# shao-lab/MotifScan

Measured on NVIDIA B200. Metric: motif_bp_scored_per_sec_both_strands, higher is better.
Workload: dtype e4m3 x e4m3 -> f16 tensor-core prefilter + f64 exact

## Files before the change

### motifscan_b200/csrc/kernels.cuh

```cuda
#pragma once
#include "common.cuh"

namespace msb {

__device__ __forceinline__ int64_t find_seq(const int64_t *__restrict__ poff, int64_t n_seqs,
                                            int64_t p) {
    int64_t lo = 0, hi = n_seqs;
    while (hi - lo > 1) {
        int64_t mid = (lo + hi) >> 1;
        if (__ldg(poff + mid) <= p) lo = mid; else hi = mid;
    }
    return lo;
}

__device__ __forceinline__ int base_code(const SeqView &S, int64_t q) {
    uint32_t m = __ldg(S.nmask + (q >> 5));
    if ((m >> (q & 31)) & 1u) return -1;
    uint32_t w = __ldg(S.codes + (q >> 4));
    return (int) ((w >> ((q & 15) * 2)) & 3u);
}

__global__ void __launch_bounds__(256)
encode_pack_kernel(const uint8_t *__restrict__ ascii, const int64_t *__restrict__ seq_off,
                   const int64_t *__restrict__ poff, const int32_t *__restrict__ len,
// ... 323 lines not shown
            const float vf = pw32[4 * c + row], vr = *(rev_end - 4 * c - row);
            if (!((w.nmask >> c) & 1u)) { f32 += vf; r32 += vr; }
        }
        if (L > left) continue;
        const float floor32 = s_floor[kl];
        const bool try_f = (E.strand & 1) && !(f32 < floor32), try_r = (E.strand & 2) && !(r32 < floor32);
        if (try_f || try_r) {
            const uint32_t m = s_motif[kl];
            const double *pw = E.mot.pwm + 4 * (int64_t) __ldg(E.mot.col_off + m);
            if (try_f) test_and_emit(E, m, p, 0, exact_raw_w(w, pw, L, 0));
            if (try_r) test_and_emit(E, m, p, 1, exact_raw_w(w, pw, L, 1));
        }
    }
}

__global__ void __launch_bounds__(256)
decode_sites_kernel(SeqView S, const uint64_t *__restrict__ key, int64_t n, int key_shift,
                    int32_t *__restrict__ seq_idx, int32_t *__restrict__ start,
                    int8_t *__restrict__ strand) {
    int64_t i = (int64_t) blockIdx.x * blockDim.x + threadIdx.x;
    if (i >= n) return;
    const uint64_t k = key[i];
    const int64_t p = site_pos(k, key_shift);
    const int64_t s = __ldg(S.blk_seq + (p >> 5));
    seq_idx[i] = (int32_t) s;
    start[i] = (int32_t) (p - __ldg(S.poff + s));
    strand[i] = (int8_t) (key_rev(k) + 1);
}

__global__ void __launch_bounds__(256)
compact_sites_kernel(const uint64_t *__restrict__ key, int64_t n, int key_shift, uint32_t *__restrict__ out) {
    const int64_t i = (int64_t) blockIdx.x * blockDim.x + threadIdx.x;
    if (i < n) out[i] = (uint32_t) (key[i] & ((1ull << key_shift) - 1ull));
}

__global__ void __launch_bounds__(256)
motif_offsets_kernel(const uint64_t *__restrict__ key, int64_t n, int32_t n_motifs, int key_shift,
                     int64_t *__restrict__ offsets) {
    const int32_t m = blockIdx.x * blockDim.x + threadIdx.x;
    if (m > n_motifs) return;
    int64_t lo = 0, hi = n;
    while (lo < hi) {
        const int64_t mid = (lo + hi) >> 1;
        if ((int64_t) site_motif(__ldg(key + mid), key_shift) < (int64_t) m) lo = mid + 1; else hi = mid;
    }
    offsets[m] = lo;
}

__global__ void __launch_bounds__(256)
count_hits_kernel(const uint64_t *__restrict__ key, int64_t n, int key_shift, int32_t n_motifs, int in_smem,
                  unsigned long long *__restrict__ counts) {
    extern __shared__ unsigned int s_hist[];
    if (in_smem) {
        for (int32_t m = threadIdx.x; m < n_motifs; m += blockDim.x) s_hist[m] = 0;
        __syncthreads();
    }
    for (int64_t i = (int64_t) blockIdx.x * blockDim.x + threadIdx.x; i < n; i += (int64_t) gridDim.x * blockDim.x) {
        const uint32_t m = site_motif(__ldg(key + i), key_shift);
        if (in_smem) atomicAdd(s_hist + m, 1u); else atomicAdd(counts + m, 1ull);
    }
    if (in_smem) {
        __syncthreads();
        for (int32_t m = threadIdx.x; m < n_motifs; m += blockDim.x)
            if (s_hist[m]) atomicAdd(counts + m, (unsigned long long) s_hist[m]);
    }
}

__global__ void __launch_bounds__(256)
region_counts_kernel(const uint64_t *__restrict__ key, const int32_t *__restrict__ seq_idx, int64_t n,
                     int key_shift, unsigned long long *__restrict__ out) {
    const int64_t i = (int64_t) blockIdx.x * blockDim.x + threadIdx.x;
    if (i >= n) return;
    const uint32_t m = site_motif(key[i], key_shift);
    if (i == 0 || site_motif(key[i - 1], key_shift) != m || seq_idx[i - 1] != seq_idx[i]) atomicAdd(out + m, 1ull);
}

__global__ void __launch_bounds__(256)
dedup_flags_kernel(const uint64_t *__restrict__ key, const int32_t *__restrict__ seq_idx,
                   const int32_t *__restrict__ start, const int8_t *__restrict__ strand,
// ... 29 lines not shown
__global__ void __launch_bounds__(256)
scatter_kept_kernel(const int32_t *__restrict__ keep, const int64_t *__restrict__ dst, int64_t n,
                    const uint64_t *__restrict__ key, const double *__restrict__ score,
                    const int32_t *__restrict__ seq_idx, const int32_t *__restrict__ start,
                    const int8_t *__restrict__ strand, uint64_t *__restrict__ o_key,
                    double *__restrict__ o_score, int32_t *__restrict__ o_seq,
                    int32_t *__restrict__ o_start, int8_t *__restrict__ o_strand) {
    const int64_t i = (int64_t) blockIdx.x * blockDim.x + threadIdx.x;
    if (i >= n || !keep[i]) return;
    const int64_t j = dst[i];
    o_key[j] = key[i];
    o_score[j] = score[i];
    o_seq[j] = seq_idx[i];
    o_start[j] = start[i];
    o_strand[j] = strand[i];
}

__global__ void __launch_bounds__(256)
score0_kernel(SeqView S, MotifView M, int strand, int32_t m_begin, int32_t m_end, int64_t out_stride,
              double *__restrict__ out) {
    const int64_t i = (int64_t) blockIdx.x * blockDim.x + threadIdx.x;
    if (i >= S.n_seqs) return;
    const int64_t p = __ldg(S.poff + i);
    for (int32_t m = m_begin + (int32_t) blockIdx.y; m < m_end; m += (int32_t) gridDim.y) {
        const int L = __ldg(M.len + m);
        const double *pw = M.pwm + 4 * (int64_t) __ldg(M.col_off + m);
        double f = 0.0, r = 0.0;
        for (int c = 0; c < L; c++) {
            const int row = base_code(S, p + c);
            if (row >= 0) {
// ... 226 lines not shown
```

### motifscan_b200/csrc/msb200.cu

```cuda
#include <cub/cub.cuh>

#include <algorithm>
#include <cmath>
#include <cstdio>
#include <cstdlib>
#include <cstring>
#include <functional>
#include <limits>
#include <mutex>
#include <new>
#include <numeric>
#include <charconv>
#include <thread>

#include "kernels.cuh"
#include "prefilter_tc.cuh"

namespace msb {

static constexpr int kSelSmemKeys = 24576;

static thread_local std::string g_err;
void set_error(const std::string &msg) { g_err = msg; }
int cuda_fail(cudaError_t e, const char *what, const char *file, int line) {
// ... 31 lines not shown
using namespace msb;

struct msb_ctx {
    int device = 0;
    cudaStream_t stream = nullptr;
    bool own_stream = false;
    int sm_count = 0;
    cudaEvent_t ev[8] = {};
    cudaStream_t copy_stream = nullptr;
    cudaEvent_t slice_ev[8] = {};
    double t[MSB_T_COUNT] = {};
    int64_t c[MSB_C_COUNT] = {};
    DevBuf ascii, seq_off, cand, dirty, hit_key, hit_score, key_alt, score_alt, sort_tmp, counters;
    DevBuf out_seq, out_start, out_strand, scores, scores_sorted, seg_off, ranks, sel;
    DevBuf keep, keep_pos, motif_counts, sel_aux, limit1;
    DevBuf lane_count;
    DevBuf bnd_range, bnd_cnt, bnd_dst, bnd_motif, bnd_seq, bnd_start, bnd_score, bnd_strand, bnd_flags;
    int64_t last_boundary = -1;
    struct FinSet {
        DevBuf key, score, seq, start, strand, offsets;
        cudaEvent_t read_done = nullptr;
        bool pending = false;
    } fin[2];
    int fin_cur = 0;
    bool last_counts_only = false;
    bool last_compact = false;
    const msb_seqs *last_seqs = nullptr;
    cudaStream_t d2h_stream = nullptr;
    cudaStream_t aux_stream = nullptr;
    cudaEvent_t aux_fork = nullptr, aux_join = nullptr;
// ... 4 lines not shown
    unsigned long long *h_counters = nullptr;
    std::vector<PinnedBlock> pinned_free;
    std::mutex pinned_mu;
    std::vector<DevBuf> dev_free;
    std::mutex dev_mu;
    int64_t last_sites = 0;
    int32_t last_n_motifs = 0;
    int64_t last_n_seqs = 0;
    int last_key_shift = 0;
    int opt_tc_prof = 0;
    int opt_ascii_slices = 4;
    int opt_tc_first_lane_cap = 0;
    int opt_poison_pool = 0;
    int opt_tc_interleave = 1;
    int opt_select_pilot = 1;
};

struct TcTableSet {
    bool valid = false;
    uint64_t cutoff_version = 0;
    std::vector<int32_t> order;
    std::vector<int32_t> slow;
    std::vector<TcBatch> batches;
    int32_t lmax_fast = 0;
    int any_zero_hit = 0;
    DevBuf d_btab, d_col_info, d_len, d_order, d_slow;
};

struct msb_motifs {
    msb_ctx *ctx = nullptr;
// ... 189 lines not shown
                  std::to_string(prop.minor));
        return MSB_ECUDA;
    }
    msb_ctx *ctx = new (std::nothrow) msb_ctx();
    if (!ctx) { set_error("out of host memory"); return MSB_ENOMEM; }
    ctx->device = device;
    ctx->sm_count = prop.multiProcessorCount;
    if (stream) {
        ctx->stream = (cudaStream_t) stream;
    } else {
        cudaError_t se = cudaStreamCreateWithFlags(&ctx->stream, cudaStreamNonBlocking);
        if (se != cudaSuccess) { delete ctx; return cuda_fail(se, "cudaStreamCreate", __FILE__, __LINE__); }
        ctx->own_stream = true;
    }
    for (auto &evt : ctx->ev) cudaEventCreate(&evt);
    cudaHostAlloc((void **) &ctx->h_counters, 4 * sizeof(unsigned long long), cudaHostAllocDefault);
    if (ctx->counters.ensure(4 * sizeof(unsigned long long)) != MSB_OK || !ctx->h_counters) {
        msb_ctx_destroy(ctx);
        return MSB_ENOMEM;
    }
    ctx->opt_tc_prof = std::getenv("MSB_TC_PROF") ? 1 : 0;
    if (cudaStreamCreateWithFlags(&ctx->aux_stream, cudaStreamNonBlocking) != cudaSuccess ||
        cudaEventCreateWithFlags(&ctx->aux_fork, cudaEventDisableTiming) != cudaSuccess ||
        cudaEventCreateWithFlags(&ctx->aux_join, cudaEventDisableTiming) != cudaSuccess) {
        cudaGetLastError();
        if (ctx->aux_stream) cudaStreamDestroy(ctx->aux_stream);
        ctx->aux_stream = nullptr;
    }
    cudaFuncSetAttribute(prefilter_tc_kernel<false>, cudaFuncAttributeMaxDynamicSharedMemorySize, kTcSmemBytes);
    cudaFuncSetAttribute(prefilter_tc_kernel<true>, cudaFuncAttributeMaxDynamicSharedMemorySize, kTcSmemBytes);
    cudaFuncSetAttribute(select_ranks_kernel<true>, cudaFuncAttributeMaxDynamicSharedMemorySize, kSelSmemKeys * 8);
    cudaFuncSetAttribute(select_ranks_kernel<false>, cudaFuncAttributeMaxDynamicSharedMemorySize, kSelSmemKeys * 8);
    *out = ctx;
    return MSB_OK;
}

int msb_ctx_destroy(msb_ctx *ctx) {
    if (!ctx) return MSB_OK;
    cudaSetDevice(ctx->device);
    cudaStreamSynchronize(ctx->stream);
    for (DevBuf *b : {&ctx->ascii, &ctx->seq_off, &ctx->cand, &ctx->dirty, &ctx->hit_key, &ctx->hit_score,
                      &ctx->key_alt, &ctx->score_alt, &ctx->sort_tmp, &ctx->counters, &ctx->out_seq,
                      &ctx->out_start, &ctx->out_strand, &ctx->scores,
                      &ctx->scores_sorted, &ctx->seg_off, &ctx->ranks, &ctx->sel, &ctx->keep, &ctx->keep_pos,
                      &ctx->motif_counts, &ctx->sel_aux, &ctx->limit1, &ctx->lane_count, &ctx->bnd_range,
                      &ctx->bnd_cnt, &ctx->bnd_dst, &ctx->bnd_motif, &ctx->bnd_seq, &ctx->bnd_start, &ctx->bnd_score,
                      &ctx->bnd_strand, &ctx->bnd_flags})
        b->release();
    if (ctx->d2h_stream) cudaStreamSynchronize(ctx->d2h_stream);
    for (auto &f : ctx->fin) {
        for (DevBuf *b : {&f.key, &f.score, &f.seq, &f.start, &f.strand, &f.offsets}) b->release();
        if (f.read_done) cudaEventDestroy(f.read_done);
    }
    if (ctx->d2h_stream) cudaStreamDestroy(ctx->d2h_stream);
    if (ctx->aux_stream) { cudaStreamSynchronize(ctx->aux_stream); cudaStreamDestroy(ctx->aux_stream); }
    if (ctx->aux_fork) cudaEventDestroy(ctx->aux_fork);
    if (ctx->aux_join) cudaEventDestroy(ctx->aux_join);
    for (auto &b : ctx->pinned_free) cudaFreeHost(b.p);
    for (auto &b : ctx->dev_free) b.release();
    if (ctx->h_counters) cudaFreeHost(ctx->h_counters);
// ... 638 lines not shown
    MSB_TRY(T.d_slow.ensure(std::max<size_t>(T.slow.size() * 4, 16)));
    cudaStream_t st = ctx->stream;
    MSB_CUDA(cudaMemcpyAsync(T.d_btab.p, btab.data(), btab.size(), cudaMemcpyHostToDevice, st));
    MSB_CUDA(cudaMemcpyAsync(T.d_col_info.p, col_info.data(), col_info.size() * 4, cudaMemcpyHostToDevice, st));
    MSB_CUDA(cudaMemcpyAsync(T.d_len.p, tc_len.data(), tc_len.size() * 4, cudaMemcpyHostToDevice, st));
    if (!fast.empty()) MSB_CUDA(cudaMemcpyAsync(T.d_order.p, fast.data(), fast.size() * 4, cudaMemcpyHostToDevice, st));
    if (!T.slow.empty()) MSB_CUDA(cudaMemcpyAsync(T.d_slow.p, T.slow.data(), T.slow.size() * 4, cudaMemcpyHostToDevice, st));
    MSB_CUDA(cudaStreamSynchronize(st));
    T.cutoff_version = M->cutoff_version;
    T.valid = true;
    *out = &T;
    return MSB_OK;
}

static int read_counters(msb_ctx *ctx) {
    MSB_CUDA(cudaMemcpyAsync(ctx->h_counters, ctx->counters.p, 4 * sizeof(unsigned long long),
                             cudaMemcpyDeviceToHost, ctx->stream));
    MSB_CUDA(cudaStreamSynchronize(ctx->stream));
    return MSB_OK;
}

static int launch_positions(msb_ctx *ctx, const ExactParams &E, const int64_t *pos, int64_t n_pos, int64_t pos_base,
                            const int32_t *ids, int32_t n_ids) {
    if (n_pos <= 0 || n_ids <= 0) return MSB_OK;
    const int64_t max_threads = (int64_t) 1 << 38;
    const int64_t pos_per_launch = std::max<int64_t>(1, max_threads / n_ids);
    for (int64_t at = 0; at < n_pos; at += pos_per_launch) {
        const int64_t cnt = std::min(pos_per_launch, n_pos - at);
        const int64_t threads = cnt * n_ids;
        ExactParams e2 = E;
        if (pos) {
            exact_positions_kernel<<<(unsigned) ((threads + 255) / 256), 256, 0, ctx->stream>>>(e2, pos + at, cnt, 0, ids, n_ids);
        } else {
            exact_positions_kernel<<<(unsigned) ((threads + 255) / 256), 256, 0, ctx->stream>>>(e2, nullptr, cnt, pos_base + at, ids, n_ids);
        }
        MSB_CUDA(cudaGetLastError());
        ctx->c[MSB_C_LAUNCHES]++;
    }
    return MSB_OK;
}

typedef std::vector<std::pair<int64_t, int64_t>> RangeList;

static int make_ranges(const msb_seqs *S, int64_t n_ranges, const int64_t *r_seq, const int64_t *r_start,
                       const int64_t *r_end, RangeList *out) {
    if (n_ranges < 0 || (n_ranges > 0 && (!r_seq || !r_start || !r_end))) { set_error("msb_scan_ranges: bad ranges"); return MSB_EINVAL; }
    out->clear();
    for (int64_t i = 0; i < n_ranges; i++) {
        if (r_seq[i] < 0 || r_seq[i] >= S->n) { set_error("msb_scan_ranges: sequence index out of range"); return MSB_EINVAL; }
        if (r_start[i] < 0) { set_error("msb_scan_ranges: negative start"); return MSB_EINVAL; }
        const int64_t slen = S->seq_off[r_seq[i] + 1] - S->seq_off[r_seq[i]];
        const int64_t a = std::min(r_start[i], slen), b = std::min(r_end[i], slen);
        if (b > a) out->push_back({S->poff[r_seq[i]] + a, S->poff[r_seq[i]] + b});
// ... 142 lines not shown
        MSB_TRY(read_counters(ctx));
        n_rec = (int64_t) ctx->h_counters[0];
        n_dirty = (int64_t) ctx->h_counters[1];
        const int64_t worst = (int64_t) ctx->h_counters[3];
        const bool overflow = worst > lane_cap;
        if (!overflow && n_dirty <= dirty_cap) break;
        if (attempt >= 2) { set_error("msb_scan: candidate buffers kept overflowing"); return MSB_ENOMEM; }
        ctx->c[MSB_C_RETRIES]++;
        if (overflow) cand_cap = std::max(cand_cap, (worst + worst / 8 + 16) * 2 * n_lanes);
        dirty_cap = std::max(dirty_cap, n_dirty + n_dirty / 16 + 1024);
        MSB_CUDA(cudaEventRecord(ctx->ev[0], st));
    }
    ctx->c[MSB_C_CANDIDATES] = n_rec;
    ctx->c[MSB_C_DIRTY] = n_dirty;

    int64_t hit_cap = std::max<int64_t>(n_rec + n_rec / 4 + 1024, 1 << 16);
    if (n_dirty) hit_cap += std::min<int64_t>(n_dirty * 2 * std::max(n_fast, 1), 1 << 24);
    if (n_slow) hit_cap += 1 << 20;
    if (ctx->hit_key.cap / 8 > (size_t) hit_cap) hit_cap = (int64_t) (ctx->hit_key.cap / 8);
    int64_t n_hits = 0;
    for (int attempt = 0;; attempt++) {
        MSB_TRY(ctx->hit_key.ensure((size_t) hit_cap * 8));
        MSB_TRY(ctx->hit_score.ensure((size_t) hit_cap * 8));
        MSB_CUDA(cudaMemsetAsync(ctx->counters.as<unsigned long long>() + 2, 0, sizeof(unsigned long long), st));
        const bool forked = ctx->aux_stream && cudaEventRecord(ctx->aux_fork, st) == cudaSuccess;
        bool join_aux = false;
        ExactParams E;
        E.seq = sv;
        E.mot = mv;
        E.strand = strand;
        E.key_shift = key_shift;
        E.hit_key = ctx->hit_key.as<uint64_t>();
        E.hit_score = ctx->hit_score.as<double>();
        E.hit_cap = hit_cap;
        E.counters = ctx->counters.as<unsigned long long>();
// ... 13 lines not shown
            }
            ctx->c[MSB_C_LAUNCHES]++;
        }
        if (n_rec) {
            exact_records_kernel<<<(unsigned) (((int64_t) n_lanes * 32 + 255) / 256), 256, 0, st>>>(
                E, ctx->cand.as<uint4>(), lane_cap, ctx->lane_count.as<uint32_t>(), n_lanes, d_order,
                TT->d_col_info.as<uint32_t>());
            MSB_CUDA(cudaGetLastError());
            ctx->c[MSB_C_LAUNCHES]++;
        }
        if (join_aux) MSB_CUDA(cudaStreamWaitEvent(st, ctx->aux_join, 0));
        if (n_slow)
            for (auto &r : *ranges)
                MSB_TRY(launch_positions(ctx, E, nullptr, r.second - r.first, r.first, d_slow, n_slow));
        MSB_CUDA(cudaEventRecord(ctx->ev[2], st));
        MSB_TRY(read_counters(ctx));
        n_hits = (int64_t) ctx->h_counters[2];
        if (n_hits <= hit_cap) break;
        if (attempt >= 2) { set_error("msb_scan: hit buffers kept overflowing"); return MSB_ENOMEM; }
        ctx->c[MSB_C_RETRIES]++;
        hit_cap = n_hits + 1024;
    }
    ctx->c[MSB_C_HITS] = n_hits;

    int64_t n_final = n_hits;
    if (counts_only) {
        MSB_TRY(ctx->motif_counts.ensure((size_t) (M->n + 1) * 8));
        MSB_CUDA(cudaMemsetAsync(ctx->motif_counts.p, 0, (size_t) (M->n + 1) * 8, st));
        if (n_hits) {
            const bool in_smem = (size_t) M->n * 4 <= 40 * 1024;
            const unsigned grid = (unsigned) std::min<int64_t>((n_hits + 2047) / 2048, (int64_t) ctx->sm_count * 8);
            count_hits_kernel<<<grid, 256, in_smem ? (size_t) M->n * 4 : 0, st>>>(
                ctx->hit_key.as<uint64_t>(), n_hits, key_shift, M->n, in_smem ? 1 : 0, ctx->motif_counts.as<unsigned long long>());
            MSB_CUDA(cudaGetLastError());
            ctx->c[MSB_C_LAUNCHES]++;
        }
        size_t scan_bytes = 0;
        MSB_CUDA(cub::DeviceScan::ExclusiveSum(nullptr, scan_bytes, ctx->motif_counts.as<int64_t>(), F.offsets.as<int64_t>(), M->n + 1, st));
        MSB_TRY(ctx->sort_tmp.ensure(std::max<size_t>(scan_bytes, 16)));
        MSB_CUDA(cub::DeviceScan::ExclusiveSum(ctx->sort_tmp.p, scan_bytes, ctx->motif_counts.as<int64_t>(), F.offsets.as<int64_t>(), M->n + 1, st));
    } else if (n_hits) {
        const bool dedup = (flags & MSB_SCAN_DEDUP) != 0;
        if ((size_t) n_hits * 25 > ((size_t) 4 << 30)) {
            msb_ctx::FinSet &O = ctx->fin[fin_set ^ 1];
            if (O.pending) { MSB_CUDA(cudaEventSynchronize(O.read_done)); O.pending = false; }
            for (DevBuf *b : {&O.key, &O.score, &O.seq, &O.start, &O.strand}) b->release();
        }
        DevBuf &s_key = dedup ? ctx->key_alt : F.key, &s_score = dedup ? ctx->score_alt : F.score;
        DevBuf &s_seq = dedup ? ctx->out_seq : F.seq, &s_start = dedup ? ctx->out_start : F.start;
        DevBuf &s_strand = dedup ? ctx->out_strand : F.strand;
        MSB_TRY(s_key.ensure((size_t) n_hits * 8));
        MSB_TRY(s_score.ensure((size_t) n_hits * 8));
        MSB_TRY(s_seq.ensure((size_t) n_hits * 4));
        MSB_TRY(s_start.ensure((size_t) n_hits * 4));
        MSB_TRY(s_strand.ensure((size_t) n_hits));
        const int end_bit = key_shift + motif_bits;
        size_t tmp_bytes = 0;
        MSB_CUDA(cub::DeviceRadixSort::SortPairs(nullptr, tmp_bytes, ctx->hit_key.as<uint64_t>(), s_key.as<uint64_t>(),
                                                 ctx->hit_score.as<double>(), s_score.as<double>(), n_hits, 0, end_bit, st));
        MSB_TRY(ctx->sort_tmp.ensure(std::max<size_t>(tmp_bytes, 16)));
        MSB_CUDA(cub::DeviceRadixSort::SortPairs(ctx->sort_tmp.p, tmp_bytes, ctx->hit_key.as<uint64_t>(), s_key.as<uint64_t>(),
                                                 ctx->hit_score.as<double>(), s_score.as<double>(), n_hits, 0, end_bit, st));
        const unsigned grid = (unsigned) ((n_hits + 255) / 256);
        const bool compact = (flags & MSB_SCAN_COMPACT) && !dedup && key_shift <= 32;
        if (compact) {
            compact_sites_kernel<<<grid, 256, 0, st>>>(s_key.as<uint64_t>(), n_hits, key_shift, s_start.as<uint32_t>());
            ctx->last_compact = true;
        } else {
            decode_sites_kernel<<<grid, 256, 0, st>>>(sv, s_key.as<uint64_t>(), n_hits, key_shift, s_seq.as<int32_t>(),
                                                      s_start.as<int32_t>(), s_strand.as<int8_t>());
        }
        MSB_CUDA(cudaGetLastError());
        ctx->c[MSB_C_LAUNCHES] += 2;
        if (dedup) {
            MSB_TRY(ctx->keep.ensure((size_t) n_hits * 4));
            MSB_TRY(ctx->keep_pos.ensure((size_t) n_hits * 8));
            MSB_TRY(F.key.ensure((size_t) n_hits * 8));
            MSB_TRY(F.score.ensure((size_t) n_hits * 8));
            MSB_TRY(F.seq.ensure((size_t) n_hits * 4));
            MSB_TRY(F.start.ensure((size_t) n_hits * 4));
            MSB_TRY(F.strand.ensure((size_t) n_hits));
            dedup_flags_kernel<<<grid, 256, 0, st>>>(s_key.as<uint64_t>(), s_seq.as<int32_t>(), s_start.as<int32_t>(),
                                                     s_strand.as<int8_t>(), s_score.as<double>(),
                                                     n_hits, mv.len, key_shift, ctx->keep.as<int32_t>());
            MSB_CUDA(cudaGetLastError());
            size_t scan_bytes = 0;
            MSB_CUDA(cub::DeviceScan::ExclusiveSum(nullptr, scan_bytes, ctx->keep.as<int32_t>(), ctx->keep_pos.as<int64_t>(), n_hits, st));
            MSB_TRY(ctx->sort_tmp.ensure(std::max<size_t>(scan_bytes, 16)));
            MSB_CUDA(cub::DeviceScan::ExclusiveSum(ctx->sort_tmp.p, scan_bytes, ctx->keep.as<int32_t>(), ctx->keep_pos.as<int64_t>(), n_hits, st));
// ... 27 lines not shown
            int64_t n_boundary = 0;
            if (boundary && cells) {
                MSB_CUDA(chains(0));
                size_t bs = 0;
                MSB_CUDA(cub::DeviceScan::ExclusiveSum(nullptr, bs, ctx->bnd_cnt.as<int64_t>(), ctx->bnd_dst.as<int64_t>(), cells + 1, st));
                MSB_TRY(ctx->sort_tmp.ensure(std::max<size_t>(bs, 16)));
                MSB_CUDA(cub::DeviceScan::ExclusiveSum(ctx->sort_tmp.p, bs, ctx->bnd_cnt.as<int64_t>(), ctx->bnd_dst.as<int64_t>(), cells + 1, st));
                MSB_CUDA(cudaMemcpyAsync(&n_boundary, ctx->bnd_dst.as<int64_t>() + cells, 8, cudaMemcpyDeviceToHost, st));
            }
            int32_t last_keep = 0;
            int64_t last_pos = 0;
            MSB_CUDA(cudaMemcpyAsync(&last_keep, ctx->keep.as<int32_t>() + (n_hits - 1), 4, cudaMemcpyDeviceToHost, st));
            MSB_CUDA(cudaMemcpyAsync(&last_pos, ctx->keep_pos.as<int64_t>() + (n_hits - 1), 8, cudaMemcpyDeviceToHost, st));
            MSB_CUDA(cudaStreamSynchronize(st));
            n_final = last_pos + last_keep;
            if (n_boundary) {
                MSB_TRY(ctx->bnd_motif.ensure((size_t) n_boundary * 4));
                MSB_TRY(ctx->bnd_seq.ensure((size_t) n_boundary * 4));
                MSB_TRY(ctx->bnd_start.ensure((size_t) n_boundary * 4));
                MSB_TRY(ctx->bnd_score.ensure((size_t) n_boundary * 8));
                MSB_TRY(ctx->bnd_strand.ensure((size_t) n_boundary));
                MSB_TRY(ctx->bnd_flags.ensure((size_t) n_boundary));
                MSB_CUDA(chains(1));
                ctx->last_boundary = n_boundary;
            }
        }
        ctx->fin_key = F.key.as<uint64_t>();
        ctx->fin_score = F.score.as<double>();
        ctx->fin_seq = F.seq.as<int32_t>();
        ctx->fin_start = F.start.as<int32_t>();
        ctx->fin_strand = F.strand.as<int8_t>();
        motif_offsets_kernel<<<(unsigned) ((M->n + 1 + 255) / 256), 256, 0, st>>>(ctx->fin_key, n_final, M->n, key_shift,
                                                                                  F.offsets.as<int64_t>());
        MSB_CUDA(cudaGetLastError());
        ctx->c[MSB_C_LAUNCHES] += 1;
    }
    MSB_CUDA(cudaEventRecord(ctx->ev[3], st));
    MSB_CUDA(cudaStreamSynchronize(st));
    ctx->t[MSB_T_PREFILTER] = ev_ms(ctx->ev[0], ctx->ev[1]);
    ctx->t[MSB_T_EXACT] = ev_ms(ctx->ev[1], ctx->ev[2]);
    ctx->t[MSB_T_ORDER] = ev_ms(ctx->ev[2], ctx->ev[3]);
    ctx->t[MSB_T_D2H] = 0;
    ctx->last_sites = n_final;
    ctx->fin_cur = fin_set;
    ctx->last_counts_only = counts_only;
    return MSB_OK;
}

}

extern "C" {

int msb_ctx_set_option(msb_ctx *ctx, const char *name, int value) {
    if (!ctx) { set_error("msb_ctx_set_option: null ctx"); return MSB_EINVAL; }
    if (name && !std::strcmp(name, "tc_prof") && (value == 0 || value == 1)) { ctx->opt_tc_prof = value; return MSB_OK; }
    if (name && !std::strcmp(name, "tc_first_lane_cap") && value >= 0) { ctx->opt_tc_first_lane_cap = value; return MSB_OK; }
    if (name && !std::strcmp(name, "ascii_slices") && value >= 1 && value <= 7) { ctx->opt_ascii_slices = value; return MSB_OK; }
    if (name && !std::strcmp(name, "poison_pool") && (value == 0 || value == 1)) { ctx->opt_poison_pool = value; return MSB_OK; }
    if (name && !std::strcmp(name, "tc_interleave") && (value == 0 || value == 1)) { ctx->opt_tc_interleave = value; return MSB_OK; }
    if (name && !std::strcmp(name, "select_pilot") && (value == 0 || value == 1)) { ctx->opt_select_pilot = value; return MSB_OK; }
    set_error("msb_ctx_set_option: unknown option or value");
    return MSB_EINVAL;
}

int msb_scan_device(msb_ctx *ctx, const msb_motifs *M, const msb_seqs *S, int strand, int flags, int64_t *n_sites) {
    MSB_TRY(scan_device(ctx, const_cast<msb_motifs *>(M), S, strand, flags));
    if (n_sites) *n_sites = ctx->last_sites;
    return MSB_OK;
}

int msb_scan_device_counts(msb_ctx *ctx, int64_t *counts, int32_t n_motifs) {
    if (!ctx || (!counts && n_motifs)) { set_error("msb_scan_device_counts: null"); return MSB_EINVAL; }
    if (n_motifs != ctx->last_n_motifs) { set_error("msb_scan_device_counts: no scan with that many motifs"); return MSB_EINVAL; }
    if (n_motifs == 0) return MSB_OK;
    MSB_CUDA(cudaSetDevice(ctx->device));
// ... 941 lines not shown
```

Before: 7121 billion.

## Replace global hit radix sort with motif-bucketed segmented block sorts

Replaces the full device radix sort of hit keys with a histogram plus bucketing pass that splits hits by motif (and sub-bins for large motifs), followed by per-segment CUB block radix sorts that also fuse site decoding. It also removes the host sync before ordering by reading the hit count on device, checking overflow afterward and retrying, and derives motif offsets from bin offsets instead of binary search. This cuts sort passes and one host round-trip, at the cost of more kernels, a fallback path for oversized segments, and possible retries when too many segments exceed block capacity.

```diff
diff --git a/motifscan_b200/csrc/kernels.cuh b/motifscan_b200/csrc/kernels.cuh
--- a/motifscan_b200/csrc/kernels.cuh
+++ b/motifscan_b200/csrc/kernels.cuh
@@ -1,4 +1,6 @@
 #pragma once
+#include <cub/block/block_radix_sort.cuh>
+
 #include "common.cuh"
 
 namespace msb {
@@ -361,55 +363,205 @@
     }
 }
 
-__global__ void __launch_bounds__(256)
-decode_sites_kernel(SeqView S, const uint64_t *__restrict__ key, int64_t n, int key_shift,
-                    int32_t *__restrict__ seq_idx, int32_t *__restrict__ start,
-                    int8_t *__restrict__ strand) {
-    int64_t i = (int64_t) blockIdx.x * blockDim.x + threadIdx.x;
-    if (i >= n) return;
-    const uint64_t k = key[i];
-    const int64_t p = site_pos(k, key_shift);
-    const int64_t s = __ldg(S.blk_seq + (p >> 5));
-    seq_idx[i] = (int32_t) s;
-    start[i] = (int32_t) (p - __ldg(S.poff + s));
-    strand[i] = (int8_t) (key_rev(k) + 1);
-}
-
-__global__ void __launch_bounds__(256)
-compact_sites_kernel(const uint64_t *__restrict__ key, int64_t n, int key_shift, uint32_t *__restrict__ out) {
-    const int64_t i = (int64_t) blockIdx.x * blockDim.x + threadIdx.x;
-    if (i < n) out[i] = (uint32_t) (key[i] & ((1ull << key_shift) - 1ull));
-}
-
-__global__ void __launch_bounds__(256)
-motif_offsets_kernel(const uint64_t *__restrict__ key, int64_t n, int32_t n_motifs, int key_shift,
+__device__ __forceinline__ int64_t hit_count(const unsigned long long *n_hits, int64_t cap) {
+    return (int64_t) min(*n_hits, (unsigned long long) cap);
+}
+
+struct BinMap {
+    const int32_t *first;
+    const int32_t *bits;
+    int key_shift;
+};
+__device__ __forceinline__ uint32_t hit_bin(const BinMap &B, uint64_t k) {
+    const uint32_t m = site_motif(k, B.key_shift);
+    if (!B.first) return m;
+    const uint64_t low = k & ((1ull << B.key_shift) - 1ull);
+    return (uint32_t) __ldg(B.first + m) + (uint32_t) (low >> (B.key_shift - __ldg(B.bits + m)));
+}
+
+__global__ void __launch_bounds__(256)
+count_hits_kernel(const uint64_t *__restrict__ key, const unsigned long long *__restrict__ n_hits, int64_t cap,
+                  BinMap B, int32_t n_bins, int in_smem, unsigned long long *__restrict__ counts) {
+    extern __shared__ unsigned int s_hist[];
+    const int64_t n = hit_count(n_hits, cap);
+    if (in_smem) {
+        for (int32_t m = threadIdx.x; m < n_bins; m += blockDim.x) s_hist[m] = 0;
+        __syncthreads();
+    }
+    for (int64_t i = (int64_t) blockIdx.x * blockDim.x + threadIdx.x; i < n; i += (int64_t) gridDim.x * blockDim.x) {
+        const uint32_t m = hit_bin(B, __ldg(key + i));
+        if (in_smem) atomicAdd(s_hist + m, 1u); else atomicAdd(counts + m, 1ull);
+    }
+    if (in_smem) {
+        __syncthreads();
+        for (int32_t m = threadIdx.x; m < n_bins; m += blockDim.x)
+            if (s_hist[m]) atomicAdd(counts + m, (unsigned long long) s_hist[m]);
+    }
+}
+
+constexpr int kSplitTarget = 8192;
+__global__ void __launch_bounds__(256)
+split_bins_kernel(const unsigned long long *__restrict__ counts, int32_t n_motifs, int key_shift,
+                  int32_t *__restrict__ bits, int32_t *__restrict__ n_bins) {
+    const int32_t m = blockIdx.x * blockDim.x + threadIdx.x;
+    if (m > n_motifs) return;
+    if (m == n_motifs) { n_bins[m] = 0; return; }
+    const unsigned long long c = counts[m];
+    int b = 0;
+    while (b < key_shift && (c >> b) > (unsigned long long) kSplitTarget) b++;
+    bits[m] = b;
+    n_bins[m] = 1 << b;
+}
+
+__global__ void __launch_bounds__(256)
+motif_offsets_kernel(const int64_t *__restrict__ bin_off, const int32_t *__restrict__ first, int32_t n_motifs,
                      int64_t *__restrict__ offsets) {
     const int32_t m = blockIdx.x * blockDim.x + threadIdx.x;
-    if (m > n_motifs) return;
-    int64_t lo = 0, hi = n;
-    while (lo < hi) {
-        const int64_t mid = (lo + hi) >> 1;
-        if ((int64_t) site_motif(__ldg(key + mid), key_shift) < (int64_t) m) lo = mid + 1; else hi = mid;
-    }
-    offsets[m] = lo;
-}
-
-__global__ void __launch_bounds__(256)
-count_hits_kernel(const uint64_t *__restrict__ key, int64_t n, int key_shift, int32_t n_motifs, int in_smem,
-                  unsigned long long *__restrict__ counts) {
-    extern __shared__ unsigned int s_hist[];
-    if (in_smem) {
-        for (int32_t m = threadIdx.x; m < n_motifs; m += blockDim.x) s_hist[m] = 0;
-        __syncthreads();
-    }
-    for (int64_t i = (int64_t) blockIdx.x * blockDim.x + threadIdx.x; i < n; i += (int64_t) gridDim.x * blockDim.x) {
-        const uint32_t m = site_motif(__ldg(key + i), key_shift);
-        if (in_smem) atomicAdd(s_hist + m, 1u); else atomicAdd(counts + m, 1ull);
-    }
-    if (in_smem) {
-        __syncthreads();
-        for (int32_t m = threadIdx.x; m < n_motifs; m += blockDim.x)
-            if (s_hist[m]) atomicAdd(counts + m, (unsigned long long) s_hist[m]);
+    if (m <= n_motifs) offsets[m] = bin_off[first[m]];
+}
+
+constexpr int kBucketThreads = 1024;
+constexpr int kBucketItems = 16;
+constexpr int kBucketTile = kBucketThreads * kBucketItems;
+__global__ void __launch_bounds__(kBucketThreads, 1)
+bucket_hits_kernel(const uint64_t *__restrict__ key, const double *__restrict__ score,
+                   const unsigned long long *__restrict__ n_hits, int64_t cap, BinMap B, int32_t n_bins,
+                   int in_smem, const int64_t *__restrict__ offsets, unsigned long long *__restrict__ fill,
+                   uint64_t *__restrict__ o_key, double *__restrict__ o_score) {
+    extern __shared__ unsigned long long s_base[];
+    unsigned int *s_cnt = (unsigned int *) (s_base + n_bins);
+    const int64_t n = hit_count(n_hits, cap);
+    if (!in_smem) {
+        for (int64_t i = (int64_t) blockIdx.x * blockDim.x + threadIdx.x; i < n; i += (int64_t) gridDim.x * blockDim.x) {
+            const uint64_t k = key[i];
+            const uint32_t m = hit_bin(B, k);
+            const int64_t dst = offsets[m] + (int64_t) atomicAdd(fill + m, 1ull);
+            o_key[dst] = k;
+            o_score[dst] = score[i];
+        }
+        return;
+    }
+    for (int64_t t0 = (int64_t) blockIdx.x * kBucketTile; t0 < n; t0 += (int64_t) gridDim.x * kBucketTile) {
+        for (int32_t m = threadIdx.x; m < n_bins; m += kBucketThreads) s_cnt[m] = 0;
+        __syncthreads();
+        uint64_t k[kBucketItems];
+        unsigned int r[kBucketItems];
+#pragma unroll
+        for (int j = 0; j < kBucketItems; j++) {
+            const int64_t i = t0 + j * kBucketThreads + threadIdx.x;
+            if (i < n) {
+                k[j] = key[i];
+                r[j] = atomicAdd(s_cnt + hit_bin(B, k[j]), 1u);
+            }
+        }
+        __syncthreads();
+        for (int32_t m = threadIdx.x; m < n_bins; m += kBucketThreads)
+            if (s_cnt[m]) s_base[m] = (unsigned long long) offsets[m] + atomicAdd(fill + m, (unsigned long long) s_cnt[m]);
+        __syncthreads();
+#pragma unroll
+        for (int j = 0; j < kBucketItems; j++) {
+            const int64_t i = t0 + j * kBucketThreads + threadIdx.x;
+            if (i < n) {
+                const int64_t dst = (int64_t) s_base[hit_bin(B, k[j])] + r[j];
+                o_key[dst] = k[j];
+                o_score[dst] = score[i];
+            }
+        }
+        __syncthreads();
+    }
+}
+
+constexpr int kMaxOversized = 32;
+__global__ void __launch_bounds__(256)
+oversized_list_kernel(const int64_t *__restrict__ offsets, int32_t n_segments, int64_t block_cap, int32_t room,
+                      int64_t *__restrict__ begin, int64_t *__restrict__ end, unsigned long long *__restrict__ n_over) {
+    const int32_t m = blockIdx.x * blockDim.x + threadIdx.x;
+    if (m < room) begin[m] = end[m] = 0;
+    __syncthreads();
+    for (int32_t s = m; s < n_segments; s += gridDim.x * blockDim.x) {
+        const int64_t a = offsets[s], b = offsets[s + 1];
+        if (b - a <= block_cap) continue;
+        const unsigned long long slot = atomicAdd(n_over, 1ull);
+        if (slot < (unsigned long long) room) { begin[slot] = a; end[slot] = b; }
+    }
+}
+
+constexpr int kOrderThreads = 1024;
+constexpr int kOrderMaxItems = 16;
+constexpr int kOrderMaxSegment = kOrderThreads * kOrderMaxItems;
+template <int ITEMS> using OrderSort = cub::BlockRadixSort<uint32_t, kOrderThreads, ITEMS, uint32_t>;
+union OrderSortStorage {
+    typename OrderSort<2>::TempStorage s2;
+    typename OrderSort<4>::TempStorage s4;
+    typename OrderSort<6>::TempStorage s6;
+    typename OrderSort<8>::TempStorage s8;
+    typename OrderSort<12>::TempStorage s12;
+    typename OrderSort<16>::TempStorage s16;
+};
+
+struct OrderParams {
+    const int64_t *offsets;
+    const uint64_t *bucket_key;
+    const double *bucket_score;
+    const uint64_t *sorted_key;
+    const double *sorted_score;
+    int64_t block_cap;
+    int key_shift;
+    int compact;
+    SeqView seq;
+    uint64_t *key;
+    double *score;
+    int32_t *seq_idx, *start;
+    int8_t *strand;
+};
+
+__device__ __forceinline__ void put_site(const OrderParams &P, int64_t i, uint64_t k, double sc) {
+    P.key[i] = k;
+    P.score[i] = sc;
+    if (P.compact) {
+        ((uint32_t *) P.start)[i] = (uint32_t) (k & ((1ull << P.key_shift) - 1ull));
+        return;
+    }
+    const int64_t p = site_pos(k, P.key_shift);
+    const int64_t s = __ldg(P.seq.blk_seq + (p >> 5));
+    P.seq_idx[i] = (int32_t) s;
+    P.start[i] = (int32_t) (p - __ldg(P.seq.poff + s));
+    P.strand[i] = (int8_t) (key_rev(k) + 1);
+}
+
+template <int ITEMS>
+__device__ __forceinline__ void order_segment_in_block(const OrderParams &P, unsigned char *smem, int64_t o, int c) {
+    const uint64_t low = (1ull << P.key_shift) - 1ull;
+    const uint64_t hi = P.bucket_key[o] & ~low;
+    uint32_t k[ITEMS], v[ITEMS];
+#pragma unroll
+    for (int j = 0; j < ITEMS; j++) {
+        const int i = threadIdx.x * ITEMS + j;
+        k[j] = i < c ? (uint32_t) (P.bucket_key[o + i] & low) : 0xffffffffu;
+        v[j] = (uint32_t) i;
+    }
+    OrderSort<ITEMS>(*reinterpret_cast<typename OrderSort<ITEMS>::TempStorage *>(smem)).SortBlockedToStriped(k, v, 0, P.key_shift);
+#pragma unroll
+    for (int j = 0; j < ITEMS; j++) {
+        const int i = j * kOrderThreads + threadIdx.x;
+        if (i < c) put_site(P, o + i, hi | k[j], P.bucket_score[o + v[j]]);
+    }
+}
+
+__global__ void __launch_bounds__(kOrderThreads, 1)
+order_segments_kernel(OrderParams P) {
+    extern __shared__ __align__(16) unsigned char order_smem[];
+    const int64_t o = P.offsets[blockIdx.x], c = P.offsets[blockIdx.x + 1] - o;
+    if (c > P.block_cap) {
+        for (int64_t i = threadIdx.x; i < c; i += kOrderThreads) put_site(P, o + i, P.sorted_key[o + i], P.sorted_score[o + i]);
+    } else if (c > 6 * kOrderThreads) {
+        if (c > 12 * kOrderThreads) order_segment_in_block<16>(P, order_smem, o, (int) c);
+        else if (c > 8 * kOrderThreads) order_segment_in_block<12>(P, order_smem, o, (int) c);
+        else order_segment_in_block<8>(P, order_smem, o, (int) c);
+    } else if (c > 0) {
+        if (c > 4 * kOrderThreads) order_segment_in_block<6>(P, order_smem, o, (int) c);
+        else if (c > 2 * kOrderThreads) order_segment_in_block<4>(P, order_smem, o, (int) c);
+        else order_segment_in_block<2>(P, order_smem, o, (int) c);
     }
 }
 
@@ -469,6 +621,15 @@
     o_seq[j] = seq_idx[i];
     o_start[j] = start[i];
     o_strand[j] = strand[i];
+}
+
+__global__ void __launch_bounds__(256)
+kept_offsets_kernel(const int64_t *__restrict__ keep_pos, int64_t n, int64_t n_final, int32_t n_motifs,
+                    int64_t *__restrict__ offsets) {
+    const int32_t m = blockIdx.x * blockDim.x + threadIdx.x;
+    if (m > n_motifs) return;
+    const int64_t o = offsets[m];
+    offsets[m] = o < n ? keep_pos[o] : n_final;
 }
 
 __global__ void __launch_bounds__(256)
diff --git a/motifscan_b200/csrc/msb200.cu b/motifscan_b200/csrc/msb200.cu
--- a/motifscan_b200/csrc/msb200.cu
+++ b/motifscan_b200/csrc/msb200.cu
@@ -69,6 +69,7 @@
     DevBuf ascii, seq_off, cand, dirty, hit_key, hit_score, key_alt, score_alt, sort_tmp, counters;
     DevBuf out_seq, out_start, out_strand, scores, scores_sorted, seg_off, ranks, sel;
     DevBuf keep, keep_pos, motif_counts, sel_aux, limit1;
+    DevBuf bin_bits, bin_first, bin_off, bucket_fill, seg_end;
     DevBuf lane_count;
     DevBuf bnd_range, bnd_cnt, bnd_dst, bnd_motif, bnd_seq, bnd_start, bnd_score, bnd_strand, bnd_flags;
     int64_t last_boundary = -1;
@@ -103,6 +104,8 @@
     int opt_poison_pool = 0;
     int opt_tc_interleave = 1;
     int opt_select_pilot = 1;
+    int opt_order_full_sort = 0;
+    int64_t opt_order_block_cap = kOrderMaxSegment;
 };
 
 struct TcTableSet {
@@ -322,8 +325,8 @@
         ctx->own_stream = true;
     }
     for (auto &evt : ctx->ev) cudaEventCreate(&evt);
-    cudaHostAlloc((void **) &ctx->h_counters, 4 * sizeof(unsigned long long), cudaHostAllocDefault);
-    if (ctx->counters.ensure(4 * sizeof(unsigned long long)) != MSB_OK || !ctx->h_counters) {
+    cudaHostAlloc((void **) &ctx->h_counters, 5 * sizeof(unsigned long long), cudaHostAllocDefault);
+    if (ctx->counters.ensure(5 * sizeof(unsigned long long)) != MSB_OK || !ctx->h_counters) {
         msb_ctx_destroy(ctx);
         return MSB_ENOMEM;
     }
@@ -339,6 +342,7 @@
     cudaFuncSetAttribute(prefilter_tc_kernel<true>, cudaFuncAttributeMaxDynamicSharedMemorySize, kTcSmemBytes);
     cudaFuncSetAttribute(select_ranks_kernel<true>, cudaFuncAttributeMaxDynamicSharedMemorySize, kSelSmemKeys * 8);
     cudaFuncSetAttribute(select_ranks_kernel<false>, cudaFuncAttributeMaxDynamicSharedMemorySize, kSelSmemKeys * 8);
+    cudaFuncSetAttribute(order_segments_kernel, cudaFuncAttributeMaxDynamicSharedMemorySize, (int) sizeof(OrderSortStorage));
     *out = ctx;
     return MSB_OK;
 }
@@ -352,6 +356,7 @@
                       &ctx->out_start, &ctx->out_strand, &ctx->scores,
                       &ctx->scores_sorted, &ctx->seg_off, &ctx->ranks, &ctx->sel, &ctx->keep, &ctx->keep_pos,
                       &ctx->motif_counts, &ctx->sel_aux, &ctx->limit1, &ctx->lane_count, &ctx->bnd_range,
+                      &ctx->bin_bits, &ctx->bin_first, &ctx->bin_off, &ctx->bucket_fill, &ctx->seg_end,
                       &ctx->bnd_cnt, &ctx->bnd_dst, &ctx->bnd_motif, &ctx->bnd_seq, &ctx->bnd_start, &ctx->bnd_score,
                       &ctx->bnd_strand, &ctx->bnd_flags})
         b->release();
@@ -1020,7 +1025,7 @@
 }
 
 static int read_counters(msb_ctx *ctx) {
-    MSB_CUDA(cudaMemcpyAsync(ctx->h_counters, ctx->counters.p, 4 * sizeof(unsigned long long),
+    MSB_CUDA(cudaMemcpyAsync(ctx->h_counters, ctx->counters.p, 5 * sizeof(unsigned long long),
                              cudaMemcpyDeviceToHost, ctx->stream));
     MSB_CUDA(cudaStreamSynchronize(ctx->stream));
     return MSB_OK;
@@ -1043,6 +1048,129 @@
         MSB_CUDA(cudaGetLastError());
         ctx->c[MSB_C_LAUNCHES]++;
     }
+    return MSB_OK;
+}
+
+static int order_hits(msb_ctx *ctx, const msb_motifs *M, const SeqView &sv, msb_ctx::FinSet &F, int key_shift,
+                      int motif_bits, int64_t hit_cap, int64_t n_hits, bool counts_only, bool dedup, bool compact) {
+    cudaStream_t st = ctx->stream;
+    const int32_t nm = M->n;
+    const unsigned long long *d_n = ctx->counters.as<unsigned long long>() + 2;
+    const unsigned hist_grid = (unsigned) std::min<int64_t>((hit_cap + 2047) / 2048, (int64_t) ctx->sm_count * 8);
+    unsigned long long *d_over = ctx->counters.as<unsigned long long>() + 4;
+    MSB_CUDA(cudaMemsetAsync(d_over, 0, sizeof(unsigned long long), st));
+    auto count_bins = [&](const BinMap &B, int32_t n_bins, DevBuf &counts, int64_t *off) -> int {
+        MSB_TRY(counts.ensure((size_t) (n_bins + 1) * 8));
+        MSB_CUDA(cudaMemsetAsync(counts.p, 0, (size_t) (n_bins + 1) * 8, st));
+        const bool in_smem = (size_t) n_bins * 4 <= 40 * 1024;
+        count_hits_kernel<<<hist_grid, 256, in_smem ? (size_t) n_bins * 4 : 0, st>>>(
+            ctx->hit_key.as<uint64_t>(), d_n, hit_cap, B, n_bins, in_smem ? 1 : 0, counts.as<unsigned long long>());
+        MSB_CUDA(cudaGetLastError());
+        size_t scan_bytes = 0;
+        MSB_CUDA(cub::DeviceScan::ExclusiveSum(nullptr, scan_bytes, counts.as<int64_t>(), off, n_bins + 1, st));
+        MSB_TRY(ctx->sort_tmp.ensure(std::max<size_t>(scan_bytes, 16)));
+        MSB_CUDA(cub::DeviceScan::ExclusiveSum(ctx->sort_tmp.p, scan_bytes, counts.as<int64_t>(), off, n_bins + 1, st));
+        ctx->c[MSB_C_LAUNCHES] += 2;
+        return MSB_OK;
+    };
+    BinMap by_motif;
+    by_motif.first = nullptr;
+    by_motif.bits = nullptr;
+    by_motif.key_shift = key_shift;
+    MSB_TRY(count_bins(by_motif, nm, ctx->motif_counts, F.offsets.as<int64_t>()));
+    if (counts_only) return MSB_OK;
+
+    DevBuf &s_key = dedup ? ctx->key_alt : F.key, &s_score = dedup ? ctx->score_alt : F.score;
+    DevBuf &s_seq = dedup ? ctx->out_seq : F.seq, &s_start = dedup ? ctx->out_start : F.start;
+    DevBuf &s_strand = dedup ? ctx->out_strand : F.strand;
+    DevBuf &b_key = dedup ? F.key : ctx->key_alt, &b_score = dedup ? F.score : ctx->score_alt;
+    MSB_TRY(s_key.ensure((size_t) hit_cap * 8));
+    MSB_TRY(s_score.ensure((size_t) hit_cap * 8));
+    MSB_TRY(s_seq.ensure((size_t) hit_cap * 4));
+    MSB_TRY(s_start.ensure((size_t) hit_cap * 4));
+    MSB_TRY(s_strand.ensure((size_t) hit_cap));
+    OrderParams P;
+    P.key_shift = key_shift;
+    P.compact = compact ? 1 : 0;
+    P.seq = sv;
+    P.key = s_key.as<uint64_t>();
+    P.score = s_score.as<double>();
+    P.seq_idx = s_seq.as<int32_t>();
+    P.start = s_start.as<int32_t>();
+    P.strand = s_strand.as<int8_t>();
+    int32_t n_segments = nm;
+    if (n_hits >= 0) {
+        size_t tmp_bytes = 0;
+        const int end_bit = key_shift + motif_bits;
+        MSB_CUDA(cub::DeviceRadixSort::SortPairs(nullptr, tmp_bytes, ctx->hit_key.as<uint64_t>(), s_key.as<uint64_t>(),
+                                                 ctx->hit_score.as<double>(), s_score.as<double>(), n_hits, 0, end_bit, st));
+        MSB_TRY(ctx->sort_tmp.ensure(std::max<size_t>(tmp_bytes, 16)));
+        MSB_CUDA(cub::DeviceRadixSort::SortPairs(ctx->sort_tmp.p, tmp_bytes, ctx->hit_key.as<uint64_t>(), s_key.as<uint64_t>(),
+                                                 ctx->hit_score.as<double>(), s_score.as<double>(), n_hits, 0, end_bit, st));
+        P.offsets = F.offsets.as<int64_t>();
+        P.bucket_key = nullptr;
+        P.bucket_score = nullptr;
+        P.sorted_key = s_key.as<uint64_t>();
+        P.sorted_score = s_score.as<double>();
+        P.block_cap = -1;
+        ctx->c[MSB_C_LAUNCHES]++;
+    } else {
+        const int64_t max_bins = (int64_t) nm + 2 * hit_cap / kSplitTarget + 1;
+        n_segments = (int32_t) max_bins;
+        MSB_TRY(ctx->bin_bits.ensure((size_t) (nm + 1) * 4));
+        MSB_TRY(ctx->bin_first.ensure((size_t) (nm + 1) * 4));
+        MSB_TRY(ctx->bin_off.ensure((size_t) (max_bins + 1) * 8));
+        MSB_TRY(ctx->seg_end.ensure((size_t) std::max<int64_t>(max_bins + 1, 2 * kMaxOversized) * 8));
+        split_bins_kernel<<<(unsigned) ((nm + 1 + 255) / 256), 256, 0, st>>>(ctx->motif_counts.as<unsigned long long>(), nm, key_shift,
+                                                                            ctx->bin_bits.as<int32_t>(), ctx->seg_end.as<int32_t>());
+        MSB_CUDA(cudaGetLastError());
+        size_t scan_bytes = 0;
+        MSB_CUDA(cub::DeviceScan::ExclusiveSum(nullptr, scan_bytes, ctx->seg_end.as<int32_t>(), ctx->bin_first.as<int32_t>(), nm + 1, st));
+        MSB_TRY(ctx->sort_tmp.ensure(std::max<size_t>(scan_bytes, 16)));
+        MSB_CUDA(cub::DeviceScan::ExclusiveSum(ctx->sort_tmp.p, scan_bytes, ctx->seg_end.as<int32_t>(), ctx->bin_first.as<int32_t>(), nm + 1, st));
+        BinMap by_bin;
+        by_bin.first = ctx->bin_first.as<int32_t>();
+        by_bin.bits = ctx->bin_bits.as<int32_t>();
+        by_bin.key_shift = key_shift;
+        MSB_TRY(count_bins(by_bin, n_segments, ctx->bucket_fill, ctx->bin_off.as<int64_t>()));
+        ctx->c[MSB_C_LAUNCHES] += 2;
+        MSB_TRY(b_key.ensure((size_t) hit_cap * 8));
+        MSB_TRY(b_score.ensure((size_t) hit_cap * 8));
+        MSB_CUDA(cudaMemsetAsync(ctx->bucket_fill.p, 0, (size_t) n_segments * 8, st));
+        const size_t bucket_smem = (size_t) n_segments * 12;
+        const bool bucket_in_smem = bucket_smem <= 48 * 1024;
+        bucket_hits_kernel<<<(unsigned) std::min<int64_t>((hit_cap + kBucketTile - 1) / kBucketTile, (int64_t) ctx->sm_count * 4),
+                             kBucketThreads, bucket_in_smem ? bucket_smem : 0, st>>>(
+            ctx->hit_key.as<uint64_t>(), ctx->hit_score.as<double>(), d_n, hit_cap, by_bin, n_segments, bucket_in_smem ? 1 : 0,
+            ctx->bin_off.as<int64_t>(), ctx->bucket_fill.as<unsigned long long>(), b_key.as<uint64_t>(), b_score.as<double>());
+        MSB_CUDA(cudaGetLastError());
+        motif_offsets_kernel<<<(unsigned) ((nm + 1 + 255) / 256), 256, 0, st>>>(ctx->bin_off.as<int64_t>(), ctx->bin_first.as<int32_t>(),
+                                                                               nm, F.offsets.as<int64_t>());
+        MSB_CUDA(cudaGetLastError());
+        const int64_t block_cap = key_shift <= 32 ? ctx->opt_order_block_cap : 0;
+        int64_t *over_begin = ctx->seg_end.as<int64_t>(), *over_end = over_begin + kMaxOversized;
+        oversized_list_kernel<<<1, 256, 0, st>>>(ctx->bin_off.as<int64_t>(), n_segments, block_cap, kMaxOversized, over_begin,
+                                                 over_end, d_over);
+        MSB_CUDA(cudaGetLastError());
+        cub::DoubleBuffer<uint64_t> dk(b_key.as<uint64_t>(), s_key.as<uint64_t>());
+        cub::DoubleBuffer<double> dv(b_score.as<double>(), s_score.as<double>());
+        size_t tmp_bytes = 0;
+        MSB_CUDA(cub::DeviceSegmentedRadixSort::SortPairs(nullptr, tmp_bytes, dk, dv, (int) hit_cap, kMaxOversized, over_begin,
+                                                          over_end, 0, key_shift, st));
+        MSB_TRY(ctx->sort_tmp.ensure(std::max<size_t>(tmp_bytes, 16)));
+        MSB_CUDA(cub::DeviceSegmentedRadixSort::SortPairs(ctx->sort_tmp.p, tmp_bytes, dk, dv, (int) hit_cap, kMaxOversized, over_begin,
+                                                          over_end, 0, key_shift, st));
+        P.offsets = ctx->bin_off.as<int64_t>();
+        P.bucket_key = b_key.as<uint64_t>();
+        P.bucket_score = b_score.as<double>();
+        P.sorted_key = dk.Current();
+        P.sorted_score = dv.Current();
+        P.block_cap = block_cap;
+        ctx->c[MSB_C_LAUNCHES] += 5;
+    }
+    order_segments_kernel<<<(unsigned) n_segments, kOrderThreads, sizeof(OrderSortStorage), st>>>(P);
+    MSB_CUDA(cudaGetLastError());
+    ctx->c[MSB_C_LAUNCHES]++;
     return MSB_OK;
 }
 
@@ -1215,11 +1343,14 @@
     ctx->c[MSB_C_CANDIDATES] = n_rec;
     ctx->c[MSB_C_DIRTY] = n_dirty;
 
+    const bool dedup = (flags & MSB_SCAN_DEDUP) != 0;
+    const bool compact = (flags & MSB_SCAN_COMPACT) && !dedup && key_shift <= 32;
     int64_t hit_cap = std::max<int64_t>(n_rec + n_rec / 4 + 1024, 1 << 16);
     if (n_dirty) hit_cap += std::min<int64_t>(n_dirty * 2 * std::max(n_fast, 1), 1 << 24);
     if (n_slow) hit_cap += 1 << 20;
     if (ctx->hit_key.cap / 8 > (size_t) hit_cap) hit_cap = (int64_t) (ctx->hit_key.cap / 8);
     int64_t n_hits = 0;
+    bool crowded = false;
     for (int attempt = 0;; attempt++) {
         MSB_TRY(ctx->hit_key.ensure((size_t) hit_cap * 8));
         MSB_TRY(ctx->hit_score.ensure((size_t) hit_cap * 8));
@@ -1263,65 +1394,41 @@
             for (auto &r : *ranges)
                 MSB_TRY(launch_positions(ctx, E, nullptr, r.second - r.first, r.first, d_slow, n_slow));
         MSB_CUDA(cudaEventRecord(ctx->ev[2], st));
-        MSB_TRY(read_counters(ctx));
-        n_hits = (int64_t) ctx->h_counters[2];
-        if (n_hits <= hit_cap) break;
-        if (attempt >= 2) { set_error("msb_scan: hit buffers kept overflowing"); return MSB_ENOMEM; }
-        ctx->c[MSB_C_RETRIES]++;
-        hit_cap = n_hits + 1024;
-    }
-    ctx->c[MSB_C_HITS] = n_hits;
-
-    int64_t n_final = n_hits;
-    if (counts_only) {
-        MSB_TRY(ctx->motif_counts.ensure((size_t) (M->n + 1) * 8));
-        MSB_CUDA(cudaMemsetAsync(ctx->motif_counts.p, 0, (size_t) (M->n + 1) * 8, st));
-        if (n_hits) {
-            const bool in_smem = (size_t) M->n * 4 <= 40 * 1024;
-            const unsigned grid = (unsigned) std::min<int64_t>((n_hits + 2047) / 2048, (int64_t) ctx->sm_count * 8);
-            count_hits_kernel<<<grid, 256, in_smem ? (size_t) M->n * 4 : 0, st>>>(
-                ctx->hit_key.as<uint64_t>(), n_hits, key_shift, M->n, in_smem ? 1 : 0, ctx->motif_counts.as<unsigned long long>());
-            MSB_CUDA(cudaGetLastError());
-            ctx->c[MSB_C_LAUNCHES]++;
-        }
-        size_t scan_bytes = 0;
-        MSB_CUDA(cub::DeviceScan::ExclusiveSum(nullptr, scan_bytes, ctx->motif_counts.as<int64_t>(), F.offsets.as<int64_t>(), M->n + 1, st));
-        MSB_TRY(ctx->sort_tmp.ensure(std::max<size_t>(scan_bytes, 16)));
-        MSB_CUDA(cub::DeviceScan::ExclusiveSum(ctx->sort_tmp.p, scan_bytes, ctx->motif_counts.as<int64_t>(), F.offsets.as<int64_t>(), M->n + 1, st));
-    } else if (n_hits) {
-        const bool dedup = (flags & MSB_SCAN_DEDUP) != 0;
-        if ((size_t) n_hits * 25 > ((size_t) 4 << 30)) {
+        if (!counts_only && (size_t) hit_cap * 25 > ((size_t) 4 << 30)) {
             msb_ctx::FinSet &O = ctx->fin[fin_set ^ 1];
             if (O.pending) { MSB_CUDA(cudaEventSynchronize(O.read_done)); O.pending = false; }
             for (DevBuf *b : {&O.key, &O.score, &O.seq, &O.start, &O.strand}) b->release();
         }
-        DevBuf &s_key = dedup ? ctx->key_alt : F.key, &s_score = dedup ? ctx->score_alt : F.score;
-        DevBuf &s_seq = dedup ? ctx->out_seq : F.seq, &s_start = dedup ? ctx->out_start : F.start;
-        DevBuf &s_strand = dedup ? ctx->out_strand : F.strand;
-        MSB_TRY(s_key.ensure((size_t) n_hits * 8));
-        MSB_TRY(s_score.ensure((size_t) n_hits * 8));
-        MSB_TRY(s_seq.ensure((size_t) n_hits * 4));
-        MSB_TRY(s_start.ensure((size_t) n_hits * 4));
-        MSB_TRY(s_strand.ensure((size_t) n_hits));
-        const int end_bit = key_shift + motif_bits;
-        size_t tmp_bytes = 0;
-        MSB_CUDA(cub::DeviceRadixSort::SortPairs(nullptr, tmp_bytes, ctx->hit_key.as<uint64_t>(), s_key.as<uint64_t>(),
-                                                 ctx->hit_score.as<double>(), s_score.as<double>(), n_hits, 0, end_bit, st));
-        MSB_TRY(ctx->sort_tmp.ensure(std::max<size_t>(tmp_bytes, 16)));
-        MSB_CUDA(cub::DeviceRadixSort::SortPairs(ctx->sort_tmp.p, tmp_bytes, ctx->hit_key.as<uint64_t>(), s_key.as<uint64_t>(),
-                                                 ctx->hit_score.as<double>(), s_score.as<double>(), n_hits, 0, end_bit, st));
-        const unsigned grid = (unsigned) ((n_hits + 255) / 256);
-        const bool compact = (flags & MSB_SCAN_COMPACT) && !dedup && key_shift <= 32;
-        if (compact) {
-            compact_sites_kernel<<<grid, 256, 0, st>>>(s_key.as<uint64_t>(), n_hits, key_shift, s_start.as<uint32_t>());
-            ctx->last_compact = true;
-        } else {
-            decode_sites_kernel<<<grid, 256, 0, st>>>(sv, s_key.as<uint64_t>(), n_hits, key_shift, s_seq.as<int32_t>(),
-                                                      s_start.as<int32_t>(), s_strand.as<int8_t>());
-        }
-        MSB_CUDA(cudaGetLastError());
-        ctx->c[MSB_C_LAUNCHES] += 2;
+        const bool full_sort = !counts_only && (ctx->opt_order_full_sort || hit_cap > (int64_t) INT32_MAX || crowded);
+        bool fits = true;
+        if (full_sort) {
+            MSB_TRY(read_counters(ctx));
+            n_hits = (int64_t) ctx->h_counters[2];
+            fits = n_hits <= hit_cap;
+        }
+        if (fits) {
+            MSB_TRY(order_hits(ctx, M, sv, F, key_shift, motif_bits, hit_cap, full_sort ? n_hits : -1, counts_only, dedup, compact));
+            MSB_CUDA(cudaEventRecord(ctx->ev[3], st));
+            if (!full_sort) {
+                MSB_TRY(read_counters(ctx));
+                n_hits = (int64_t) ctx->h_counters[2];
+                fits = n_hits <= hit_cap;
+                if (fits && ctx->h_counters[4] > (unsigned long long) kMaxOversized) { fits = false; crowded = true; }
+            }
+        }
+        if (fits) break;
+        if (attempt >= 2) { set_error("msb_scan: hit buffers kept overflowing"); return MSB_ENOMEM; }
+        ctx->c[MSB_C_RETRIES]++;
+        hit_cap = std::max(hit_cap, n_hits + 1024);
+    }
+    ctx->c[MSB_C_HITS] = n_hits;
+
+    int64_t n_final = n_hits;
+    if (!counts_only && n_hits) {
         if (dedup) {
+            DevBuf &s_key = ctx->key_alt, &s_score = ctx->score_alt, &s_seq = ctx->out_seq, &s_start = ctx->out_start;
+            DevBuf &s_strand = ctx->out_strand;
+            const unsigned grid = (unsigned) ((n_hits + 255) / 256);
             MSB_TRY(ctx->keep.ensure((size_t) n_hits * 4));
             MSB_TRY(ctx->keep_pos.ensure((size_t) n_hits * 8));
             MSB_TRY(F.key.ensure((size_t) n_hits * 8));
@@ -1379,6 +1486,10 @@
             MSB_CUDA(cudaMemcpyAsync(&last_pos, ctx->keep_pos.as<int64_t>() + (n_hits - 1), 8, cudaMemcpyDeviceToHost, st));
             MSB_CUDA(cudaStreamSynchronize(st));
             n_final = last_pos + last_keep;
+            kept_offsets_kernel<<<(unsigned) ((M->n + 1 + 255) / 256), 256, 0, st>>>(ctx->keep_pos.as<int64_t>(), n_hits, n_final,
+                                                                                     M->n, F.offsets.as<int64_t>());
+            MSB_CUDA(cudaGetLastError());
+            ctx->c[MSB_C_LAUNCHES]++;
             if (n_boundary) {
                 MSB_TRY(ctx->bnd_motif.ensure((size_t) n_boundary * 4));
                 MSB_TRY(ctx->bnd_seq.ensure((size_t) n_boundary * 4));
@@ -1389,19 +1500,16 @@
                 MSB_CUDA(chains(1));
                 ctx->last_boundary = n_boundary;
             }
+            MSB_CUDA(cudaEventRecord(ctx->ev[3], st));
+            MSB_CUDA(cudaStreamSynchronize(st));
         }
         ctx->fin_key = F.key.as<uint64_t>();
         ctx->fin_score = F.score.as<double>();
         ctx->fin_seq = F.seq.as<int32_t>();
         ctx->fin_start = F.start.as<int32_t>();
         ctx->fin_strand = F.strand.as<int8_t>();
-        motif_offsets_kernel<<<(unsigned) ((M->n + 1 + 255) / 256), 256, 0, st>>>(ctx->fin_key, n_final, M->n, key_shift,
-                                                                                  F.offsets.as<int64_t>());
-        MSB_CUDA(cudaGetLastError());
-        ctx->c[MSB_C_LAUNCHES] += 1;
-    }
-    MSB_CUDA(cudaEventRecord(ctx->ev[3], st));
-    MSB_CUDA(cudaStreamSynchronize(st));
+        ctx->last_compact = compact;
+    }
     ctx->t[MSB_T_PREFILTER] = ev_ms(ctx->ev[0], ctx->ev[1]);
     ctx->t[MSB_T_EXACT] = ev_ms(ctx->ev[1], ctx->ev[2]);
     ctx->t[MSB_T_ORDER] = ev_ms(ctx->ev[2], ctx->ev[3]);
@@ -1424,6 +1532,8 @@
     if (name && !std::strcmp(name, "poison_pool") && (value == 0 || value == 1)) { ctx->opt_poison_pool = value; return MSB_OK; }
     if (name && !std::strcmp(name, "tc_interleave") && (value == 0 || value == 1)) { ctx->opt_tc_interleave = value; return MSB_OK; }
     if (name && !std::strcmp(name, "select_pilot") && (value == 0 || value == 1)) { ctx->opt_select_pilot = value; return MSB_OK; }
+    if (name && !std::strcmp(name, "order_full_sort") && (value == 0 || value == 1)) { ctx->opt_order_full_sort = value; return MSB_OK; }
+    if (name && !std::strcmp(name, "order_block_cap") && value >= 0 && value <= kOrderMaxSegment) { ctx->opt_order_block_cap = value; return MSB_OK; }
     set_error("msb_ctx_set_option: unknown option or value");
     return MSB_EINVAL;
 }
```

After: 6996 billion (median of 6 runs). -1.7%, worse.
